# yukw777/EILEV

Hardware: AMD Instinct MI355X
Metric: clips/sec (8-frame, 16 in-context) encode+generate, eilev-blip2-opt-2.7b (higher is better)
Workload: dtype bf16

## Files before the change

eilev_amd/csrc/attention.hip:

```cpp
#include <type_traits>

#include "common.h"
#include <type_traits>
#include <utility>

int g_attn_force_v1 = 0, g_attn_dbg = 0;
#ifdef EILEV_PROBES
extern "C" int eilev_debug_attn_v1(int on) { g_attn_force_v1 = on & 1; g_attn_dbg = on >> 1; return 0; }
#endif

namespace {

template <int DP, bool DROP = false>
__global__ __launch_bounds__(256) void attn_prefill_kernel(const AttnArgs a) {
    constexpr int KD = DP / 32;
    constexpr int DT = DP / 16;
    constexpr int CH = DP / 8;
    constexpr int KSTR = DP * 2 + 16;
    constexpr int VSTR = 64 * 2 + 16;
    __shared__ __attribute__((aligned(16))) char ks_[64 * KSTR];
    __shared__ __attribute__((aligned(16))) char vt_[DP * VSTR];
    __shared__ int msk_[64];

    const int tid = threadIdx.x, lane = tid & 63, wid = tid >> 6;
// ... 157 lines not shown
template <int NWQ, int DB = 3, bool REL = false>
__global__ __launch_bounds__(64 * NWQ) void attn_prefill_v2_kernel(const AttnArgs a) {
    constexpr int KD = 2 * DB;
    constexpr bool SWZ = DB == 2;
    extern __shared__ __attribute__((aligned(16))) char smem[];
    const int RS = DB == 4 ? 272 : a.hd * 2, CH = RS >> 4;
    const int CHS = a.hd >> 3;
    const int T = 64 * RS;
    int *msk = reinterpret_cast<int *>(smem + 4 * T + 256);
    float *rel_lds = reinterpret_cast<float *>(smem + attn_v2_rel_offset(NWQ, a.hd));

    const int tid = threadIdx.x, lane = tid & 63;
    const int wid = __builtin_amdgcn_readfirstlane(tid >> 6);
    const int l31 = lane & 31, hi = lane >> 5;
    const int b = blockIdx.z, h = blockIdx.y;
    const int q0 = (blockIdx.x * NWQ + wid) * 32;
    const int qrow = q0 + l31;
    const int off = a.skv - a.sq;
    const float sl2 = a.scale * 1.44269504088896340736f;

    const bf16 *qp = a.q + (int64_t)b * a.q_bs + (int64_t)h * a.q_hs;
    const bf16 *kp = a.k + (int64_t)b * a.k_bs + (int64_t)h * a.k_hs;
    const bf16 *vp = a.v + (int64_t)b * a.v_bs + (int64_t)h * a.v_hs;

    int kv_end = a.skv;
    if (a.causal) {
        const int last_q = min(a.sq - 1, (int)(blockIdx.x * NWQ + NWQ) * 32 - 1);
        kv_end = min(a.skv, last_q + off + 1);
    }
    const int ntiles = (kv_end + 63) / 64;

    auto stage_in = [&](int buf, int t) {
        const int kv0 = t * 64;
        for (int i = wid; i < 2 * CH; i += NWQ) {
            const bool isv = i >= CH;
            const int pi = isv ? i - CH : i;
            const int pch = pi * 64 + lane, key = pch / CH, cl = pch - key * CH;
            const int c = SWZ ? (cl ^ ((key >> 1) & 7)) : (DB == 4 && cl >= CHS ? CHS - 1 : cl);
            int gk = kv0 + key;
            gk = gk < a.skv ? gk : a.skv - 1;
            const bf16 *src = isv ? vp + (int64_t)gk * a.ldv + c * 8 : kp + (int64_t)gk * a.ldk + c * 8;
            char *dst = smem + buf * 2 * T + (isv ? T : 0) + pi * 1024;
// ... 121 lines not shown
#pragma unroll
                for (int db = 0; db < DB; ++db) {
                    const char *va = vbase + (kb * 32 + 16 * s2) * RS + (SWZ ? 0 : db * 64);
                    const bf16x4 lo = __builtin_amdgcn_ds_read_tr16_b64_v4bf16((lds_bf16x4_t *)(va + (SWZ ? db * 64 : 0)));
                    const bf16x4 hi4 = __builtin_amdgcn_ds_read_tr16_b64_v4bf16((lds_bf16x4_t *)(va + 8 * RS + (SWZ ? (db ^ 1) * 64 : 0)));
                    const bf16x8 vf = {lo[0], lo[1], lo[2], lo[3], hi4[0], hi4[1], hi4[2], hi4[3]};
                    o[db] = __builtin_amdgcn_mfma_f32_32x32x16_bf16(vf, pb, o[db], 0, 0, 0);
                }
            }
        }
    };

    for (int t = 0; t < ntiles; ++t) {
        const int cur = t & 1;
        if (t + 1 < ntiles && !(a.dbg & DBG_ATTN_NO_PREFETCH)) stage_in(cur ^ 1, t + 1);
        if (active && !(a.dbg & DBG_ATTN_NO_COMPUTE)) {
            const int kv0 = t * 64;
            int vis_end = kv_end;
            if (a.causal) vis_end = min(vis_end, min(a.sq - 1, q0 + 31) + off + 1);
            const bool plain = msk[128 + cur] != 0 && (!a.causal || kv0 + 63 <= q0 + off);
            using two = std::integral_constant<int, 2>;
            using one = std::integral_constant<int, 1>;
            if (NWQ > 8 || (DB == 4 && NWQ == 8)) {
                if (kv0 < vis_end) {
                    if (plain) tile_body(one{}, std::false_type{}, cur, kv0);
                    else tile_body(one{}, std::true_type{}, cur, kv0);
                }
                if (kv0 + 32 < vis_end) {
                    if (plain) tile_body(one{}, std::false_type{}, cur, kv0 + 32);
                    else tile_body(one{}, std::true_type{}, cur, kv0 + 32);
// ... 309 lines not shown
}

template <int HD, int NT>
int launch_attn_frame(const AttnArgs &a, hipStream_t s) {
    constexpr int CH = HD / 8;
    constexpr int NPIECE = (NT * 16 * CH + (12 - CH) + 63) / 64;
    constexpr int smem = 3 * NPIECE * 1024;
    const int npairs = a.batch * a.heads;
    const int grid = npairs < eilev_grid_cus() ? npairs : eilev_grid_cus();
    return eilev_launch<attn_frame_kernel<HD, NT>>(dim3(grid), dim3(576), smem, s, a);
}

#include "attn_frame3.h"

template <int NWQ, int DB = 3, bool REL = false>
int launch_attn_v2(const AttnArgs &a, hipStream_t s) {
    size_t smem = attn_v2_rel_offset(NWQ, a.hd) + (REL ? (size_t)(a.rel_n + 2 * ATTN_V2_REL_SLACK) * sizeof(float) : 0);
    const dim3 grid((a.sq + 32 * NWQ - 1) / (32 * NWQ), a.heads, a.batch), block(64 * NWQ);
    return eilev_launch<attn_prefill_v2_kernel<NWQ, DB, REL>>(grid, block, smem, s, a);
}

}

int launch_attention(const AttnArgs &a_in, hipStream_t s) {
    AttnArgs a = a_in;
    a.dbg = g_attn_dbg;
    if (a.batch <= 0 || a.sq <= 0) return EILEV_OK;
    if (!a.q || !a.k || !a.v || !a.o || a.skv <= 0) return EILEV_E_BADARG;
    if ((a.hd & 7) || a.hd > 128 || (a.ldq & 7) || (a.ldk & 7) || (a.ldv & 7) || (a.ldo & 7) || ((uintptr_t)a.o & 15) || (a.q_hs & 7) ||
        (a.k_hs & 7) || (a.v_hs & 7) || (a.o_hs & 7) || (a.q_bs & 7) || (a.k_bs & 7) || (a.v_bs & 7) || (a.o_bs & 7))
        return EILEV_E_UNSUPPORTED;
    if (a.hm) {
        if (a.hd != 88 || a.sq != 257 || a.skv != 257 || a.causal || a.key_mask || a.rel_tab || a.drop_thr || (a.q_hs & 7) || (a.q_bs & 7) ||
// ... 49 lines not shown
```

eilev_amd/csrc/common.h:

```cpp
#pragma once
#include <hip/hip_runtime.h>
#include <stdint.h>

#include <type_traits>

#include "../../include/eilev.h"

typedef __bf16 bf16;
typedef __attribute__((ext_vector_type(8))) __bf16 bf16x8;
typedef __attribute__((ext_vector_type(4))) __bf16 bf16x4;
typedef __attribute__((ext_vector_type(2))) __bf16 bf16x2;
typedef __attribute__((ext_vector_type(4))) float f32x4;
typedef __attribute__((ext_vector_type(16))) float f32x16;

#define EILEV_HIP_CHECK(expr)                          \
    do {                                               \
        hipError_t _e = (expr);                        \
        if (_e != hipSuccess) return (int)_e;          \
    } while (0)

static inline int eilev_num_cu() {
    static int n = 0;
    if (!n) {
        int dev = 0, cu = 0;
// ... 219 lines not shown
    DBG_ATTN_FRAME_STAMPS = 1 << 8,
    DBG_ATTN_FRAME3_STAMPS = 1 << 9,
    DBG_ATTN_HEAD_MAJOR = 1 << 10,
    DBG_ATTN_FRAME3_NO_STORES = 1 << 11,
};
enum GemmForce : int { FORCE_NONE = 0, FORCE_PP4 = 9, FORCE_W6 = 12, FORCE_64x128 = 13, FORCE_128x128 = 14, FORCE_SPLIT_K = 15 };

struct GemmArgs {
    const bf16 *A;
    int64_t lda;
    const bf16 *W;
    int64_t ldw;
    const bf16 *Wp = nullptr;
    int a_frag = 0, c_frag = 0, ln_frag = 0;
    int hm_tok = 0, hm_heads = 0, hm_hd = 0;
    const bf16 *bias;
    const bf16 *resid;
    int64_t ldr;
    void *C;
    int64_t ldc;
    int M, N, K;
    int epi;
    int out_f32;
    float scale;
    int scale_cols;
    int patch_group;
    int dbg;
    float *scratch;
    size_t scratch_bytes;
    const float *wscale = nullptr;
// ... 5 lines not shown
    const float *ln_csum = nullptr;
    float *stat_out = nullptr;
    int64_t stat_ld = 0;
    const bf16 *ln_gamma = nullptr, *ln_beta = nullptr;
    bf16 *ln_out = nullptr;
    float ln_eps = 0.0f;
    int k_slice = 0;
    unsigned long long *trace = nullptr;
    int trace_tiles = 0;
};

__host__ __device__ static inline int64_t frag32_index(int row, int col) { return (int64_t)(col >> 5) * 1024 + row * 32 + (col & 31); }

int launch_gemm(const GemmArgs &g, int prof_kind, hipStream_t s);
bool gemm_rows32_takes(const GemmArgs &g);
int launch_pp4_ext(const GemmArgs &g, int grid, hipStream_t s);
#ifdef EILEV_PROBES
#define EILEV_TRACE_M16 true
#else
#define EILEV_TRACE_M16 false
#endif
static inline bool pp4_all_lean(const GemmArgs &g) {
    const bool scale_ok = g.scale_cols == 0 || (g.scale_cols % 16 == 0 && g.epi == 0 && !g.resid && !g.ln_rows && !g.stat_out);
    return g.N % 128 == 0 && !g.out_f32 && g.patch_group == 0 && scale_ok && !g.wscale && !g.ascale && !g.dbg && (!g.trace || EILEV_TRACE_M16);
}
static inline bool hm_takes(const GemmArgs &g) {
    return g.hm_tok > 0 && g.hm_heads > 0 && g.hm_hd > 64 && g.hm_hd % 8 == 0 && g.N == 3 * g.hm_heads * g.hm_hd && g.ln_rows && g.epi == 0 && !g.resid &&
           !g.stat_out && !g.scale_cols && pp4_all_lean(g) && g.N % 64 == 0 && g.M % g.hm_tok == 0 && (int64_t)g.M * g.N * 2 < 0xfffffff0ll;
}
bool gemv_rows_ok(int M, int N, int K);
int launch_gemv_rows(int pro, const bf16 *x, int64_t ldx, const bf16 *gamma, const bf16 *beta, float eps, const float *part, int heads, int hd,
                     int nsplit, const bf16 *W, const bf16 *bias, const bf16 *resid, int64_t ldr, void *out, int64_t ldo, int out_f32, int M, int N,
                     int K, int epi, float scale, int scale_cols, hipStream_t s);
bool gemv1_ok(int N, int K, int pro);
int launch_gemv1(int pro, const bf16 *x, const bf16 *gamma, const bf16 *beta, float eps, const bf16 *W, const bf16 *bias, const bf16 *resid, void *out,
                 int out_f32, int N, int K, int epi, float scale, int scale_cols, hipStream_t s, const float *part = nullptr, int heads = 0, int hd = 0,
                 int nsplit = 0);
bool gemvm_ok(int M, int N, int K, int pro);
int launch_gemvm(int pro, const bf16 *x, int64_t ldx, const bf16 *gamma, const bf16 *beta, float eps, const bf16 *W, const bf16 *bias, const bf16 *resid,
                 int64_t ldr, void *out, int64_t ldo, int out_f32, int M, int N, int K, int epi, float scale, int scale_cols, hipStream_t s);
int launch_im2col(const void *pix, int dtype, bf16 *out, int64_t rows, int frames, int img, int patch, int kp, hipStream_t s);
int launch_pad_rows(const bf16 *w, bf16 *out, int rows, int k, int kp, hipStream_t s);
int launch_cls_rows(const bf16 *cls, const bf16 *pos, bf16 *x, int64_t frames_total, int tok, int d, hipStream_t s);
int launch_quant_rows_e4m3(const bf16 *x, int64_t ldx, uint8_t *q, float *scale, int64_t rows, int cols, hipStream_t s);
// ... 30 lines not shown
    const bf16 *q, *k, *v;
    bf16 *o;
    int64_t q_bs, k_bs, v_bs, o_bs;
    int64_t q_hs, k_hs, v_hs, o_hs;
    int64_t ldq, ldk, ldv, ldo;
    int batch, heads, sq, skv, hd;
    float scale;
    int causal;
    const int32_t *key_mask;
    int64_t mask_ld;
    int dbg = 0;
    const float *rel_tab = nullptr;
    int64_t rel_hs = 0;
    int rel_off = 0, rel_n = 0;
    int hm = 0;
    uint32_t drop_thr = 0, drop_seed = 0;
    float drop_scale = 1.0f;
};
static inline AttnArgs attn_rows(const bf16 *q, int64_t ldq, const bf16 *k, int64_t ldk, const bf16 *v, int64_t ldv, bf16 *o, int64_t batch,
                                 int64_t heads, int64_t sq, int64_t skv, int64_t hd, float scale) {
    AttnArgs a;
    a.q = q; a.k = k; a.v = v; a.o = o;
    a.q_bs = sq * ldq; a.k_bs = skv * ldk; a.v_bs = skv * ldv; a.o_bs = sq * heads * hd;
    a.q_hs = a.k_hs = a.v_hs = a.o_hs = hd;
    a.ldq = ldq; a.ldk = ldk; a.ldv = ldv; a.ldo = heads * hd;
    a.batch = (int)batch; a.heads = (int)heads; a.sq = (int)sq; a.skv = (int)skv; a.hd = (int)hd; a.scale = scale; a.causal = 0;
    a.key_mask = nullptr; a.mask_ld = 0;
    return a;
}
static inline AttnArgs attn_cache(const bf16 *q, int64_t ldq, const bf16 *kplane, const bf16 *vplane, int64_t cap, bf16 *o, int64_t batch,
// ... 38 lines not shown
```

eilev_amd/csrc/gemm.hip:

```cpp
#include "gemm_common.h"
#include "gemm_tiled.h"
#include "gemm_pp4.h"
#include "gemm_w6.h"
#include "gemm_skinny.h"

int g_eilev_grid_cus = 0;
#ifdef EILEV_PROBES
int g_gemm_debug = 0;
extern "C" int eilev_debug_gemm_flags(int f) { g_gemm_debug = f; return 0; }
extern "C" int eilev_debug_grid_cus(int n) { g_eilev_grid_cus = n; return 0; }
#endif
#ifdef EILEV_PROBES
unsigned long long *g_gemm_trace = nullptr;
int g_gemm_trace_tiles = 0;
extern "C" int eilev_debug_gemm_trace(void *buf, int tiles) { g_gemm_trace = (unsigned long long *)buf; g_gemm_trace_tiles = tiles; return 0; }
#endif

namespace {

#ifndef EILEV_A3_MIN_K
#define EILEV_A3_MIN_K 5120
#endif
bool a3_takes(const GemmArgs &g) { return g.epi == 0 && g.K >= EILEV_A3_MIN_K; }

int launch_pp4(const GemmArgs &g, hipStream_t s) {
    constexpr int smem = PP4_SMEM;
    const int tiles = ((g.M + 255) / 256) * ((g.N + 255) / 256);
    const int ncu = eilev_grid_cus();
    const int grid = tiles < ncu ? tiles : ncu / 8 * 8;
    if (g.A8 || g.ln_rows || g.stat_out) return launch_pp4_ext(g, grid, s);
    if (pp4_all_lean(g) && g.epi != 1) {
        if (a3_takes(g)) return eilev_launch<gemm_pp4_kernel<0, false, 0, 2, true>>(dim3(grid), dim3(512), smem, s, g);
        return eilev_with_epi<0, 2>(g.epi, [&](auto e) { return eilev_launch<gemm_pp4_kernel<decltype(e)::value, false, 0, 2>>(dim3(grid), dim3(512), smem, s, g); });
    }
    return eilev_with_epi<0, 1, 2>(g.epi, [&](auto e) { return eilev_launch<gemm_pp4_kernel<decltype(e)::value>>(dim3(grid), dim3(512), smem, s, g); });
}

constexpr int64_t kOffsetLimit = 0x7fff0000ll;
bool fits_offset(int64_t rows, int64_t ld) { return rows * ld * 2 < kOffsetLimit; }

GemmArgs with_probes(const GemmArgs &g_in) {
    GemmArgs g = g_in;
#ifdef EILEV_PROBES
    g.dbg = g_gemm_debug;
    g.trace = g_gemm_trace;
    g.trace_tiles = g_gemm_trace_tiles;
// ... 27 lines not shown
bool w8_streams(const GemmArgs &g) { return g.M <= 32 && g.K % 256 == 0 && g.patch_group == 0; }
int w8_check(const GemmArgs &g) {
    if (!g.A || !g.C || !g.wscale || g.N <= 0 || g.K <= 0 || g.ldw != g.K || ((uintptr_t)g.W8 & 15) || (g.K & 15)) return EILEV_E_BADARG;
    if (!w8_streams(g) && !g.w8_scratch) return EILEV_E_WORKSPACE;
    return EILEV_OK;
}
int w8_expand(const GemmArgs &g, hipStream_t s) {
    const int64_t n16 = (int64_t)g.N * g.K / 16;
    hipLaunchKernelGGL(w8_expand_kernel, dim3((unsigned)ceil_div64(n16, 256)), dim3(256), 0, s, g.W8, g.w8_scratch, n16);
    EILEV_LAUNCH_CHECK();
    return EILEV_OK;
}

bool ln_fold(const GemmArgs &g) { return g.ln_rows != nullptr || g.stat_out != nullptr; }
bool skinny_dma_ok(const GemmArgs &g) { return g.K % 256 == 0 && (!(g.dbg & DBG_GEMM_SKINNY_NO_DMA) || g.W8); }
bool skinny_takes(const GemmArgs &g) { return (g.M <= 16 || (g.M <= 32 && skinny_dma_ok(g))) && g.patch_group == 0 && !ln_fold(g); }

int check_args(const GemmArgs &g) {
    if (!g.A || !g.W || !g.C || g.N <= 0 || g.K <= 0) return EILEV_E_BADARG;
    if ((g.K & 7) || (g.lda & 7) || (g.ldw & 7) || ((uintptr_t)g.A & 15) || ((uintptr_t)g.W & 15)) return EILEV_E_UNSUPPORTED;
    if (g.hm_tok && (!hm_takes(g) || !fits_offset(g.M, g.lda))) return EILEV_E_UNSUPPORTED;
    if (ln_fold(g) && (g.W8 || g.wscale || g.out_f32 || g.patch_group || g.scale_cols || g.K % BK || !fits_offset(g.N, g.ldw))) return EILEV_E_UNSUPPORTED;
    const bool skinny = skinny_takes(g);
    if ((g.a_frag || g.c_frag || g.ln_frag) && !skinny) return EILEV_E_UNSUPPORTED;
    if (!skinny && !g.out_f32 && ((g.ldc & 7) || (g.N & 3) || ((uintptr_t)g.C & 15) || (g.resid && ((g.ldr & 7) || ((uintptr_t)g.resid & 15))) ||
                                   (g.bias && ((uintptr_t)g.bias & 7))))
        return EILEV_E_UNSUPPORTED;
    return EILEV_OK;
}


// ... 125 lines not shown
}
int launch_split_k(const GemmArgs &g, hipStream_t s) {
    const int tiles = (int)(ceil_div64(g.M, 128) * ceil_div64(g.N, 128)), nk = g.K / BK;
    int slices = 512 / tiles;
    slices = slices < 2 ? 2 : (slices > 16 ? 16 : slices);
    if (slices > nk / 8) slices = nk / 8 > 1 ? nk / 8 : 1;
    GemmArgs gs = g;
    gs.k_slice = (nk + slices - 1) / slices;
    slices = (nk + gs.k_slice - 1) / gs.k_slice;
    EILEV_HIP_CHECK(hipMemsetAsync(g.C, 0, (size_t)g.M * g.ldc * sizeof(float), s));
    return eilev_launch<gemm_glds_kernel<128, 128, 2, 2, 0, 2, 2, 0>>(dim3(tiles, slices), dim3(256), 2 * (128 + 128) * 128, s, gs);
}

bool t64x128_takes(const GemmArgs &g) { return ceil_div64(g.M, 128) * ceil_div64(g.N, 128) < 96 && g.M > 64; }

int launch_wide(const GemmArgs &g, hipStream_t s) {
    const int force = (g.dbg >> DBG_GEMM_FORCE_SHIFT) & 15;
    const bool no_dma = g.dbg & DBG_GEMM_NO_DMA;
    int cfg = tile_cfg(g);
    bool promoted = false;
    if (cfg == CFG_256x128_1S && g.K % BK == 0 && !(g.dbg & DBG_GEMM_NO_WIDE)) cfg = CFG_256x256, promoted = true;
    if (cfg == CFG_256x128 && w6_ok(g) && force == FORCE_NONE && !(g.dbg & (DBG_GEMM_NO_WIDE | DBG_GEMM_NO_W6 | DBG_GEMM_NO_DMA))) cfg = CFG_256x256, promoted = true;
    if (force == FORCE_PP4) cfg = CFG_256x256;
    if (force == FORCE_64x128 || force == FORCE_128x128 || force == FORCE_SPLIT_K) cfg = CFG_128x128;
    else if (force >= CFG_256x256 && force <= CFG_128x128) cfg = force;

    if (w6_ok(g) && (force == FORCE_W6 || (force == FORCE_NONE && cfg == CFG_256x256 && w6_pick(g) && !(g.dbg & (DBG_GEMM_NO_W6 | DBG_GEMM_NO_DMA)))))
        return launch_w6(g, s);
    switch (cfg) {
        case CFG_256x256:
            if (!(promoted && (g.dbg & DBG_GEMM_WIDE_TILED)) && (force == FORCE_NONE || force == FORCE_PP4) && !no_dma && g.K % BK == 0 && fits_offset(g.N, g.ldw))
                return launch_pp4(g, s);
            return launch_tiled<256, 256, 2, 4, 2, 2>(g, s);
        case CFG_256x128_1S: return launch_tiled<256, 128, 4, 2, 1, 4, 1>(g, s);
        case CFG_256x128: return launch_tiled<256, 128, 4, 2, 2, 2>(g, s);
        default:
            if (split_k_takes(g) && (force == FORCE_NONE || force == FORCE_SPLIT_K) && !no_dma) return launch_split_k(g, s);
            if ((force == FORCE_64x128 || (force == FORCE_NONE && t64x128_takes(g))) && g.M > 64 && !no_dma) return launch_tiled<64, 128, 1, 2, 2, 3>(g, s);
            return launch_tiled<128, 128, 2, 2, 2, 2>(g, s);
    }
}

}


static int launch_gemm_core(const GemmArgs &g_in, int prof_kind, hipStream_t s, bool *ln_done);

bool gemm_rows32_takes(const GemmArgs &g) {
    if (!g.A || !g.W || !g.C || g.W8 || g.wscale || g.M <= 16 || g.M > 32 || g.K % 256 || g.patch_group || g.ln_rows || g.stat_out) return false;
    if ((g.lda & 7) || (g.ldw & 7) || ((uintptr_t)g.A & 15) || ((uintptr_t)g.W & 15) || (g.dbg & DBG_GEMM_NO_ROWS32)) return false;
    SkinnyArgs a;
    a.g = g;
    a.mr = 32;
    int ks = 1, ksteps = 0, grid_x = 0;
    return rows32_plan(g, (g.N + 15) / 16, skinny_n_cu(), a, ks, ksteps, grid_x);
}

extern "C" int eilev_stream_layout_pack(const void *w, int64_t n, int64_t k, void *out, void *stream) {
    if (!w || !out || w == out || n < 1 || k < 1) return EILEV_E_BADARG;
    if (n > 0x7fffffff || k > 0x7fffffff || n * k > 0x7fffffff0ll) return EILEV_E_UNSUPPORTED;
    int ks = 0, ksteps = 0, grid_x = 0;
    if (!rows32_shape((int)n, (int)k, skinny_n_cu(), ks, ksteps, grid_x)) return EILEV_E_UNSUPPORTED;
    const int64_t chunks = n * (k >> 3);
    hipLaunchKernelGGL(stream_pack_kernel, dim3((unsigned)((chunks + 255) / 256)), dim3(256), 0, (hipStream_t)stream, (const bf16 *)w, (bf16 *)out, (int)n, (int)k, grid_x);
    EILEV_LAUNCH_CHECK();
    return EILEV_OK;
}

int launch_gemm(const GemmArgs &g, int prof_kind, hipStream_t s) {
    bool ln_done = false;
    const int rc = launch_gemm_core(g, prof_kind, s, &ln_done);
// ... 10 lines not shown
    if (g.W8) {
        const int rc = w8_check(g);
        if (rc != EILEV_OK) return rc;
        if (!w8_streams(g)) {
            const int rc_x = w8_expand(g, s);
            if (rc_x != EILEV_OK) return rc_x;
            GemmArgs e = g_in;
            e.W = g.w8_scratch;
            e.W8 = nullptr;
            return launch_gemm_core(e, prof_kind, s, ln_done);
        }
        g.W = reinterpret_cast<const bf16 *>(g.W8);
    }
    const int rc = check_args(g);
    if (rc != EILEV_OK) return rc;
    if (skinny_takes(g)) return launch_skinny(g, s, ln_done);
    if (const int64_t rows = chunk_rows(g)) return launch_row_chunks(g_in, rows, prof_kind, s);
    return profiled(ln_fold(g) ? launch_pp4 : launch_wide, g, prof_kind, s);
}
```

eilev_amd/csrc/gemm_pp4.h:

```cpp
#pragma once
#include "gemm_common.h"

namespace {

#ifndef EILEV_PP4_DEEP
#define EILEV_PP4_DEEP 1
#endif
template <int EPI, bool F8 = false, int LN = 0, int M16K = 0, bool A3 = false>
__global__ __launch_bounds__(512, 2) void gemm_pp4_kernel(const GemmArgs g) {
    constexpr bool M16 = M16K != 0, HT16 = M16K == 2;
    static_assert(!M16 || !F8, "16 x 16 form: bf16 instances");
    constexpr int BM = 256, BN = 256, NWM = 2, NWN = 4, NW = 8;
    constexpr int WM = BM / NWM, WN = BN / NWN, TM = WM / 32, TN = WN / 32;
    constexpr int STEP = (BM + BN) * 128;
    constexpr int PC = 8;
    static_assert(!A3 || M16, "A3: lean epilogues only");
    constexpr int STG0 = A3 ? 2 * BM * 128 : 2 * STEP;

    extern __shared__ __attribute__((aligned(16))) char smem[];
    auto a_slot = [&](int st) { return smem + (A3 ? (st % 3) * (BM * 128) : (st & 1) * STEP); };
    auto w_slot = [&](int st) { return smem + (A3 ? 3 * (BM * 128) + (st & 1) * (BN * 128) : (st & 1) * STEP + BM * 128); };
    const int tiles_m = (g.M + BM - 1) / BM, tiles_n = (g.N + BN - 1) / BN, ntiles = tiles_m * tiles_n;
    const int tid = threadIdx.x, lane = tid & 63;
    const int wid = __builtin_amdgcn_readfirstlane(tid >> 6);
    const int wm = wid / NWN, wn = wid % NWN;
    const int l31 = lane & 31, hi = lane >> 5;
// ... 229 lines not shown
                } else {
                    const int cph = (HD - 64) >> 3, jb = ((rr - NH * 64) >> 3) + schunk, hh = jb / cph;
                    ent.x = (plane * NH + hh) * TOK * HD + TOK * 64 + (jb - hh * cph) * 8;
                    ent.y = HD - 64;
                }
                const int fw = __builtin_amdgcn_readfirstlane(r0 / TOK);
                const int m0 = r0 + srow, f0 = m0 / TOK;
                hm_t = m0 - f0 * TOK;
                hm_str2 = __builtin_amdgcn_readfirstlane(ent.y * 2);
                hm_off = (unsigned)(((f0 - fw) * TOK * g.N + ent.x + hm_t * ent.y) * 2);
                hm_off_w = hm_off + (unsigned)(TOK * g.N * 2) - (unsigned)(TOK * hm_str2);
                const int64_t left = ((int64_t)g.M / TOK - fw) * TOK * g.N * 2;
                rch = uniform_rsrc(reinterpret_cast<bf16 *>(g.C) + (int64_t)fw * TOK * g.N, (int)(unsigned)(left < 0xfffffff0ll ? left : 0xfffffff0ll));
            }
        }
        u32x4_t rv[4];
        auto res_load = [&](int u) {
#pragma unroll
            for (int it = 0; it < 4; ++it) rv[it] = __builtin_amdgcn_raw_buffer_load_b128(rr, rs_voff, (u * 32 + it * 8) * (int)(g.ldr * 2), 0);
        };
        if constexpr (RES) res_load(0);
        bf16x4 biasr[M16 ? 1 : TN][4];
        bf16x4 biasr16[M16 ? TN16 : 1];
        if constexpr (M16) {
#pragma unroll
            for (int j = 0; j < TN16; ++j) {
                if (g.bias) biasr16[j] = *reinterpret_cast<const bf16x4 *>(g.bias + cn0 + coff + j * 16 + g4 * 4);
                else biasr16[j] = (bf16x4){(bf16)0.f, (bf16)0.f, (bf16)0.f, (bf16)0.f};
            }
        } else {
// ... 125 lines not shown
                }
            } else if constexpr (LNP) {
                typedef __attribute__((ext_vector_type(2))) unsigned u32x2_t;
                const f32x2_t t = (f32x2_t){st1 + __shfl_xor(st1, 32), st2 + __shfl_xor(st2, 32)};
                if (hi == 0) __builtin_amdgcn_raw_buffer_store_b64(__builtin_bit_cast(u32x2_t, t), rst, (U * 32 + l31) * 8, 0, 0);
            }
            __builtin_amdgcn_sched_barrier(0);
            bf16x8 erb[2];
#pragma unroll
            for (int h2 = 0; h2 < 2; ++h2) {
#pragma unroll
                for (int b = 0; b < 2; ++b) {
                    const int row = (h2 * 2 + b) * 8 + srow;
                    erb[b] = *reinterpret_cast<const bf16x8 *>(stg + row * 128 + ((schunk ^ (row & 7)) << 4));
                }
                if (hm) {
                    if constexpr (HMI) {
#pragma unroll
                        for (int b = 0; b < 2; ++b) {
                            const int RO = U * 32 + (h2 * 2 + b) * 8;
                            const unsigned vo = hm_t + RO >= g.hm_tok ? hm_off_w : hm_off;
                            __builtin_amdgcn_raw_buffer_store_b128(__builtin_bit_cast(u32x4_t, erb[b]), rch, vo, RO * hm_str2, EILEV_HM_AUX);
                        }
                    }
                } else {
#pragma unroll
                for (int b = 0; b < 2; ++b)
                    __builtin_amdgcn_raw_buffer_store_b128(__builtin_bit_cast(u32x4_t, erb[b]), rc, st_voff, (U * 32 + (h2 * 2 + b) * 8) * (int)(g.ldc * 2), EILEV_ST_AUX);
                }
            }
            asm volatile("s_nop 1" ::: "memory");
            __builtin_amdgcn_sched_barrier(0);
        });
    };
#define PP_WAIT_LGKM0() __builtin_amdgcn_s_waitcnt(0xC07F)
#define PP_WAIT_LGKM0_VM0() __builtin_amdgcn_s_waitcnt(0x0070)
// ... 265 lines not shown
```

eilev_amd/csrc/misc.hip:

```cpp
#include "common.h"

namespace {

template <typename T>
__global__ void im2col_kernel(const T *__restrict__ pix, bf16 *__restrict__ out, int64_t rows, int frames, int img,
                              int patch, int kp) {
    const int64_t idx = (int64_t)blockIdx.x * blockDim.x + threadIdx.x;
    const int chunks = kp >> 3;
    if (idx >= rows * chunks) return;
    const int64_t row = idx / chunks;
    const int c = (int)(idx - row * chunks);
    const int g = img / patch, gg = g * g, pp = patch * patch;
    const int64_t f = row / gg;
    const int p = (int)(row - f * gg), py = p / g, px = p - py * g;
    const int64_t n = f / frames;
    const int t = (int)(f - n * frames);
    float v[8];
#pragma unroll
    for (int e = 0; e < 8; ++e) {
        const int k = c * 8 + e;
        float val = 0.0f;
        if (k < 3 * pp) {
            const int ch = k / pp, rem = k - ch * pp, dy = rem / patch, dx = rem - dy * patch;
            val = (float)pix[(((n * 3 + ch) * frames + t) * img + py * patch + dy) * (int64_t)img + px * patch + dx];
// ... 667 lines not shown
                     int past) {
    hipLaunchKernelGGL(pos_ids_kernel, dim3(batch), dim3(1024), 0, s, mask, pid, L);
    EILEV_LAUNCH_CHECK();
    hipLaunchKernelGGL(add_pos_kernel, dim3(batch * (L - past)), dim3(256), 0, s, emb, pos, pid, h, d, L - past, L, past);
    EILEV_LAUNCH_CHECK();
    return EILEV_OK;
}
int launch_decode_embed(const bf16 *embed, const bf16 *pos, const int64_t *tokens, const int32_t *n_valid, const int32_t *state,
                        int vocab, int max_pid, bf16 *h, int batch, int d, hipStream_t s) {
    hipLaunchKernelGGL(decode_embed_kernel, dim3(batch), dim3(256), 0, s, embed, pos, tokens, n_valid, state, vocab, max_pid, h, d);
    EILEV_LAUNCH_CHECK();
    return EILEV_OK;
}
int launch_kv_write(const bf16 *qkv, bf16 *kc, bf16 *vc, int batch, int rows_per_b, int heads, int hd, int cap, int seq_len,
                    const int32_t *state, hipStream_t s, int slot0) {
    hipLaunchKernelGGL(kv_write_kernel, dim3(batch * rows_per_b), dim3(256), 0, s, qkv, kc, vc, rows_per_b, heads, hd, cap, seq_len, state, slot0);
    EILEV_LAUNCH_CHECK();
    return EILEV_OK;
}
int launch_topk_logprob(const float *logits, const float *row_score, int rows, int vocab, int keep, float *out_val, int32_t *out_idx, hipStream_t s) {
    if (vocab > 65536 || (vocab & 3) || keep < 1 || keep > 64 || (((uintptr_t)logits) & 15)) return EILEV_E_UNSUPPORTED;
    hipLaunchKernelGGL(topk_logprob_kernel, dim3(rows), dim3(1024), 0, s, logits, row_score, vocab, keep, out_val, out_idx);
    EILEV_LAUNCH_CHECK();
    return EILEV_OK;
}
int launch_beam_advance(const float *row_lp, const int32_t *row_tok, int batch, int beams, int keep, int max_new, const int32_t *state,
                        const int64_t *eos_ids, int n_eos, const float *len_pow, int recip, int early, int64_t *run_seq, float *run_score,
                        int64_t *fin_seq, float *fin_score, int64_t *fin_len, uint8_t *finished, uint8_t *can_improve, int64_t *tokens, int32_t *anc,
                        int gen_cap, int64_t *scratch, hipStream_t s) {
    if (beams * keep > 2048 || keep > 64 || beams > 32 || (anc && gen_cap * beams > 32 * 64) || n_eos > 8) return EILEV_E_UNSUPPORTED;
    BeamAdvanceArgs a;
// ... 210 lines not shown
```

eilev_amd/csrc/opt.hip:

```cpp
#include "stages.h"

namespace {
inline int64_t opt_ws_rows(int64_t M) { return (M > 16 && M < 32) ? 32 : M; }

struct OptBufs {
    bf16 *h, *x, *att, *qkv, *ffn;
    int32_t *pid;
    float *scratch;
    uint8_t *a8;
    float *a8_scale;
    size_t used;
};

OptBufs carve_opt(const EilevDims *d, int64_t M, void *ws) {
    Carver cv{(char *)ws};
    OptBufs b;
    M = opt_ws_rows(M);
    b.h = cv.take<bf16>((size_t)M * d->t_hidden);
    b.x = cv.take<bf16>((size_t)M * d->t_hidden);
    b.att = cv.take<bf16>((size_t)M * d->t_hidden);
    b.qkv = cv.take<bf16>((size_t)M * 3 * d->t_hidden);
    b.ffn = cv.take<bf16>((size_t)M * d->t_ffn);
    b.pid = cv.take<int32_t>((size_t)M);
    b.scratch = cv.take<float>(kSkinnyScratch / sizeof(float));
// ... 23 lines not shown
        g.W8 = w8;
        g.wscale = sc;
        g.ldw = g.K;
        return EILEV_OK;
    }
    if (g.M > 32 || g.K % 256 != 0) {
        if (!w->w8_expand || w->w8_expand_bytes < (size_t)g.N * g.K * sizeof(bf16)) return EILEV_E_WORKSPACE;
        g.w8_scratch = (bf16 *)w->w8_expand;
    }
    g.W8 = w8;
    g.wscale = sc;
    g.ldw = g.K;
    return EILEV_OK;
}

int opt_qkv(const EilevDims *d, const EilevOptWeights *w, int l, const OptBufs &b, int64_t M, hipStream_t s, int a_frag = 0) {
    const EilevOptLayer *L = &w->layers[l];
    const int D = d->t_hidden;
    const float scaling = 1.0f / sqrtf((float)(D / d->t_heads));
    const void *ws[3] = {L->q_w, L->k_w, L->v_w}, *bs[3] = {L->q_b, L->k_b, L->v_b};
    const bool bias_fused = packed(bs, 3, D);
    if (w->layers_w8) {
        if (!bias_fused && (L->q_b || L->k_b || L->v_b)) return EILEV_E_UNSUPPORTED;
        GemmArgs g = sk_gemm(b.scratch, b.x, D, nullptr, D, L->q_b, nullptr, 0, b.qkv, 3 * D, M, 3 * D, D, 0);
        g.scale = scaling; g.scale_cols = D;
        RC(use_w8(g, w, w->layers_w8[l].qkv_w8, w->layers_w8[l].qkv_scale, b, s));
        return launch_gemm(g, 5, s);
    }
    const bool fused = packed(ws, 3, (size_t)D * D) && bias_fused;
    for (int i = 0; i < (fused ? 1 : 3); ++i) {
        GemmArgs g = sk_gemm(b.scratch, b.x, D, ws[i], D, bs[i], nullptr, 0, b.qkv + i * D, 3 * D, M, fused ? 3 * D : D, D, 0);
        if (i == 0) { g.scale = scaling; g.scale_cols = D; }
        if (fused && w->layers_stream && M > 16 && M <= 32) g.Wp = (const bf16 *)w->layers_stream[l].qkv_s;
        g.a_frag = a_frag;
        RC(launch_gemm(g, 5, s));
    }
    return EILEV_OK;
}

int opt_tail(const EilevDims *d, const EilevOptWeights *w, int l, const OptBufs &b, int64_t M, hipStream_t s, const void *next_ln_w = nullptr,
             const void *next_ln_b = nullptr, int frag = 0, bool dry = false) {
    const EilevOptLayer *L = &w->layers[l];
    const EilevOptLayerW8 *Q = w->layers_w8 ? &w->layers_w8[l] : nullptr;
    const int D = d->t_hidden, Ft = d->t_ffn;
    const EilevOptLayerStream *S = (w->layers_stream && !Q && M > 16 && M <= 32) ? &w->layers_stream[l] : nullptr;
    GemmArgs g = sk_gemm(b.scratch, b.att, D, L->o_w, D, L->o_b, b.h, D, b.h, D, M, D, D, 0);
    g.ln_gamma = (const bf16 *)L->ln2_w; g.ln_beta = (const bf16 *)L->ln2_b; g.ln_out = b.x; g.ln_eps = d->t_eps;
    if (S) g.Wp = (const bf16 *)S->o_s;
    g.a_frag = g.ln_frag = frag;
// ... 6 lines not shown
    if (dry && !gemm_rows32_takes(g)) return EILEV_E_UNSUPPORTED;
    if (Q) RC(use_w8(g, w, Q->fc1_w8, Q->fc1_scale, b, s));
    if (!dry) RC(launch_gemm(g, 5, s));
    g = sk_gemm(b.scratch, b.ffn, Ft, L->fc2_w, Ft, L->fc2_b, b.h, D, b.h, D, M, D, Ft, 0);
    if (S) g.Wp = (const bf16 *)S->fc2_s;
    if (next_ln_w) {
        g.ln_gamma = (const bf16 *)next_ln_w; g.ln_beta = (const bf16 *)next_ln_b; g.ln_out = b.x; g.ln_eps = d->t_eps;
    }
    g.a_frag = frag;
    g.ln_frag = next_ln_w ? frag : 0;
    if (dry) return gemm_rows32_takes(g) ? EILEV_OK : EILEV_E_UNSUPPORTED;
    if (Q) RC(use_w8(g, w, Q->fc2_w8, Q->fc2_scale, b, s));
    return launch_gemm(g, 5, s);
}

int g_decode_frag = 1;
}
int g_decode_rows = 1;
#ifdef EILEV_PROBES
extern "C" int eilev_debug_decode_rows(int on) { g_decode_rows = on; return 0; }
extern "C" int eilev_debug_decode_frag(int on) { g_decode_frag = on; return 0; }
#endif
namespace {

bool opt_qkv_packed(const EilevDims *d, const EilevOptWeights *w) {
    const int D = d->t_hidden;
    for (int l = 0; l < d->t_layers; ++l) {
        const EilevOptLayer *L = &w->layers[l];
        const void *ws[3] = {L->q_w, L->k_w, L->v_w}, *bs[3] = {L->q_b, L->k_b, L->v_b};
        if (!packed(ws, 3, (size_t)D * D) || !L->q_b || !packed(bs, 3, D)) return false;
// ... 98 lines not shown
        const EilevOptLayer *L = &w->layers[l];
        DecodeAttnArgs al = at_block(a, l, kv_layer, gen_layer);
        al.out_frag = frag;
        if (l == 0) RC(launch_layernorm(b.h, D, (const bf16 *)L->ln1_w, (const bf16 *)L->ln1_b, b.x, D, M, D, d->t_eps, s));
        RC(opt_qkv(d, w, l, b, M, s, l > 0 ? frag : 0));
        RC(launch_attn_decode(al, s));
        const bool last = l + 1 == d->t_layers;
        RC(opt_tail(d, w, l, b, M, s, last ? w->final_ln_w : w->layers[l + 1].ln1_w, last ? w->final_ln_b : w->layers[l + 1].ln1_b, frag));
    }
    GemmArgs g = opt_lm_head(d, w, b, M, logits);
    g.a_frag = frag;
    return launch_gemm(g, 5, s);
}

int opt_blocks(const EilevDims *d, const EilevOptWeights *w, const OptBufs &b, const void *inputs_embeds, const int32_t *attn_mask, int64_t batch,
               int64_t rows, int64_t past_len, bool from_cache, void *kv_cache, int64_t kv_capacity, void *hidden, hipStream_t s) {
    const int D = d->t_hidden, H = d->t_heads, hd = D / H;
    const int64_t M = batch * rows, total = past_len + rows;
    RC(launch_pos_embed((const bf16 *)inputs_embeds, (const bf16 *)w->embed_positions, attn_mask, b.pid, b.h, (int)batch, (int)total, D,
                        s, (int)past_len));
    const KvCache kv(batch, D, kv_capacity);
    const size_t hs_bytes = (size_t)M * D * sizeof(bf16);
    for (int l = 0; l < d->t_layers; ++l) {
        const EilevOptLayer *L = &w->layers[l];
        bf16 *kc = kv.k((bf16 *)kv_cache, l), *vc = kv.v((bf16 *)kv_cache, l);
        if (hidden) RC(copy_hidden(hidden, l, b.h, hs_bytes, s));
        RC(launch_layernorm(b.h, D, (const bf16 *)L->ln1_w, (const bf16 *)L->ln1_b, b.x, D, M, D, d->t_eps, s));
        RC(opt_qkv(d, w, l, b, M, s));
        RC(launch_kv_write(b.qkv, kc, vc, (int)batch, (int)rows, H, hd, (int)kv_capacity, (int)total, nullptr, s, (int)past_len));
        AttnArgs a = from_cache ? attn_cache(b.qkv, 3 * D, kc, vc, kv_capacity, b.att, batch, H, rows, total, hd, 1.0f)
                                : attn_rows(b.qkv, 3 * D, b.qkv + D, 3 * D, b.qkv + 2 * D, 3 * D, b.att, batch, H, rows, total, hd, 1.0f);
        a.causal = 1; a.key_mask = attn_mask; a.mask_ld = total;
        RC(launch_attention(a, s));
        RC(opt_tail(d, w, l, b, M, s));
    }
    RC(launch_layernorm(b.h, D, (const bf16 *)w->final_ln_w, (const bf16 *)w->final_ln_b, b.x, D, M, D, d->t_eps, s));
    if (hidden) RC(copy_hidden(hidden, d->t_layers, b.x, hs_bytes, s));
    return EILEV_OK;
}

int opt_prefill_impl(const EilevDims *d, const EilevOptWeights *w, const void *inputs_embeds, const int32_t *attn_mask, int64_t batch,
                     int64_t seq_len, void *kv_cache, int64_t kv_capacity, float *logits_last, float *logits_all, void *hidden,
                     void *workspace, size_t workspace_bytes, void *stream) {
    if (!d || !w || !inputs_embeds || !attn_mask || !kv_cache || !workspace || batch <= 0 || seq_len <= 0) return EILEV_E_BADARG;
    if (seq_len > kv_capacity || seq_len > d->max_pos) return EILEV_E_BADARG;
    if (!dims_ok_opt(d)) return EILEV_E_UNSUPPORTED;
    if (workspace_bytes < eilev_opt_workspace_bytes(d, batch, seq_len)) return EILEV_E_WORKSPACE;
    hipStream_t s = (hipStream_t)stream;
    const int D = d->t_hidden;
    const int64_t M = batch * seq_len;
    const OptBufs b = carve_opt(d, M, workspace);
    RC(opt_blocks(d, w, b, inputs_embeds, attn_mask, batch, seq_len, 0, false, kv_cache, kv_capacity, hidden, s));
    if (logits_all) {
        GemmArgs g = mk_gemm(b.x, D, w->embed_tokens, D, nullptr, nullptr, 0, logits_all, d->vocab, M, d->vocab, D, 0);
        g.out_f32 = 1;
        RC(launch_gemm(g, 5, s));
    }
    if (logits_last) {
        GemmArgs g = sk_gemm(b.scratch, b.x + (seq_len - 1) * (int64_t)D, seq_len * (int64_t)D, w->embed_tokens, D, nullptr, nullptr, 0,
                             logits_last, d->vocab, batch, d->vocab, D, 0);
        g.out_f32 = 1;
        RC(launch_gemm(g, 5, s));
    }
    return EILEV_OK;
}
}

// ... 155 lines not shown
```

Before: 231.7.

## Fuse KV-cache write into QKV GEMM and compute last layer only for final row

Adds a KVC epilogue to the pp4 QKV GEMM that writes the K and V planes straight into the KV cache, so prefill no longer needs the separate kv_write kernel. In the last OPT layer it runs attention only for the final query block and does out-proj, LN2 and the FFN only on each sample's last row, since only last-row logits are needed. The attention kernel also zeroes masked K/V rows in LDS, because values now come from the cache, and it gains a query-block offset. In exchange it adds complex eligibility checks and a new GEMM instance, and it risks correctness because cache rows are read directly.

Result: no change. 232.4 (median of 6 runs) (+0.3%).

```diff
diff --git a/eilev_amd/csrc/attention.hip b/eilev_amd/csrc/attention.hip
--- a/eilev_amd/csrc/attention.hip
+++ b/eilev_amd/csrc/attention.hip
@@ -195,7 +195,8 @@
     const int wid = __builtin_amdgcn_readfirstlane(tid >> 6);
     const int l31 = lane & 31, hi = lane >> 5;
     const int b = blockIdx.z, h = blockIdx.y;
-    const int q0 = (blockIdx.x * NWQ + wid) * 32;
+    const int qblk = blockIdx.x + a.qb0;
+    const int q0 = (qblk * NWQ + wid) * 32;
     const int qrow = q0 + l31;
     const int off = a.skv - a.sq;
     const float sl2 = a.scale * 1.44269504088896340736f;
@@ -206,7 +207,7 @@
 
     int kv_end = a.skv;
     if (a.causal) {
-        const int last_q = min(a.sq - 1, (int)(blockIdx.x * NWQ + NWQ) * 32 - 1);
+        const int last_q = min(a.sq - 1, (qblk * NWQ + NWQ) * 32 - 1);
         kv_end = min(a.skv, last_q + off + 1);
     }
     const int ntiles = (kv_end + 63) / 64;
@@ -358,6 +359,17 @@
     for (int t = 0; t < ntiles; ++t) {
         const int cur = t & 1;
         if (t + 1 < ntiles && !(a.dbg & DBG_ATTN_NO_PREFETCH)) stage_in(cur ^ 1, t + 1);
+        if (msk[128 + cur] == 0) {
+            char *kt = smem + cur * 2 * T;
+            for (int i = tid; i < 64 * CH; i += 64 * NWQ) {
+                const int key = i / CH, c16 = (i - key * CH) * 16;
+                if (!msk[cur * 64 + key]) {
+                    *reinterpret_cast<uint4 *>(kt + key * RS + c16) = make_uint4(0, 0, 0, 0);
+                    *reinterpret_cast<uint4 *>(kt + T + key * RS + c16) = make_uint4(0, 0, 0, 0);
+                }
+            }
+            __syncthreads();
+        }
         if (active && !(a.dbg & DBG_ATTN_NO_COMPUTE)) {
             const int kv0 = t * 64;
             int vis_end = kv_end;
@@ -697,9 +709,12 @@
 #include "attn_frame3.h"
 
 template <int NWQ, int DB = 3, bool REL = false>
-int launch_attn_v2(const AttnArgs &a, hipStream_t s) {
+int launch_attn_v2(const AttnArgs &a_in, hipStream_t s) {
+    AttnArgs a = a_in;
+    const int qblocks = (a.sq + 32 * NWQ - 1) / (32 * NWQ);
+    a.qb0 = a.last_q_only ? qblocks - 1 : 0;
     size_t smem = attn_v2_rel_offset(NWQ, a.hd) + (REL ? (size_t)(a.rel_n + 2 * ATTN_V2_REL_SLACK) * sizeof(float) : 0);
-    const dim3 grid((a.sq + 32 * NWQ - 1) / (32 * NWQ), a.heads, a.batch), block(64 * NWQ);
+    const dim3 grid(qblocks - a.qb0, a.heads, a.batch), block(64 * NWQ);
     return eilev_launch<attn_prefill_v2_kernel<NWQ, DB, REL>>(grid, block, smem, s, a);
 }
 
diff --git a/eilev_amd/csrc/common.h b/eilev_amd/csrc/common.h
--- a/eilev_amd/csrc/common.h
+++ b/eilev_amd/csrc/common.h
@@ -257,6 +257,9 @@
     const bf16 *Wp = nullptr;
     int a_frag = 0, c_frag = 0, ln_frag = 0;
     int hm_tok = 0, hm_heads = 0, hm_hd = 0;
+    bf16 *kvc_k = nullptr, *kvc_v = nullptr;
+    int kvc_rows = 0, kvc_cap = 0, kvc_heads = 0, kvc_hd = 0;
+    int family_pp4 = 0;
     const bf16 *bias;
     const bf16 *resid;
     int64_t ldr;
@@ -292,6 +295,7 @@
 
 int launch_gemm(const GemmArgs &g, int prof_kind, hipStream_t s);
 bool gemm_rows32_takes(const GemmArgs &g);
+bool gemm_wide_on_pp4(const GemmArgs &g);
 int launch_pp4_ext(const GemmArgs &g, int grid, hipStream_t s);
 #ifdef EILEV_PROBES
 #define EILEV_TRACE_M16 true
@@ -306,6 +310,13 @@
     return g.hm_tok > 0 && g.hm_heads > 0 && g.hm_hd > 64 && g.hm_hd % 8 == 0 && g.N == 3 * g.hm_heads * g.hm_hd && g.ln_rows && g.epi == 0 && !g.resid &&
            !g.stat_out && !g.scale_cols && pp4_all_lean(g) && g.N % 64 == 0 && g.M % g.hm_tok == 0 && (int64_t)g.M * g.N * 2 < 0xfffffff0ll;
 }
+static inline bool kvc_takes(const GemmArgs &g) {
+    const int64_t w = (int64_t)g.kvc_heads * g.kvc_hd;
+    return g.kvc_k && g.kvc_v && g.kvc_heads > 0 && g.kvc_hd > 0 && g.kvc_hd % 8 == 0 && w % 64 == 0 && g.N == 3 * w && g.kvc_rows >= 128 &&
+           g.kvc_rows <= g.kvc_cap && g.M % g.kvc_rows == 0 && g.epi == 0 && !g.resid && !g.ln_rows && !g.stat_out && !g.ln_out && !g.hm_tok &&
+           pp4_all_lean(g) && 2 * w * g.kvc_cap * 2 < 0xfffffff0ll;
+}
+bool gemm_kvc_takes(const GemmArgs &g);
 bool gemv_rows_ok(int M, int N, int K);
 int launch_gemv_rows(int pro, const bf16 *x, int64_t ldx, const bf16 *gamma, const bf16 *beta, float eps, const float *part, int heads, int hd,
                      int nsplit, const bf16 *W, const bf16 *bias, const bf16 *resid, int64_t ldr, void *out, int64_t ldo, int out_f32, int M, int N,
@@ -366,6 +377,7 @@
     int64_t rel_hs = 0;
     int rel_off = 0, rel_n = 0;
     int hm = 0;
+    int last_q_only = 0, qb0 = 0;
     uint32_t drop_thr = 0, drop_seed = 0;
     float drop_scale = 1.0f;
 };
diff --git a/eilev_amd/csrc/gemm.hip b/eilev_amd/csrc/gemm.hip
--- a/eilev_amd/csrc/gemm.hip
+++ b/eilev_amd/csrc/gemm.hip
@@ -30,6 +30,7 @@
     const int grid = tiles < ncu ? tiles : ncu / 8 * 8;
     if (g.A8 || g.ln_rows || g.stat_out) return launch_pp4_ext(g, grid, s);
     if (pp4_all_lean(g) && g.epi != 1) {
+        if (g.kvc_k) return eilev_launch<gemm_pp4_kernel<0, false, 0, 2, false, true>>(dim3(grid), dim3(512), smem, s, g);
         if (a3_takes(g)) return eilev_launch<gemm_pp4_kernel<0, false, 0, 2, true>>(dim3(grid), dim3(512), smem, s, g);
         return eilev_with_epi<0, 2>(g.epi, [&](auto e) { return eilev_launch<gemm_pp4_kernel<decltype(e)::value, false, 0, 2>>(dim3(grid), dim3(512), smem, s, g); });
     }
@@ -87,7 +88,7 @@
 
 bool ln_fold(const GemmArgs &g) { return g.ln_rows != nullptr || g.stat_out != nullptr; }
 bool skinny_dma_ok(const GemmArgs &g) { return g.K % 256 == 0 && (!(g.dbg & DBG_GEMM_SKINNY_NO_DMA) || g.W8); }
-bool skinny_takes(const GemmArgs &g) { return (g.M <= 16 || (g.M <= 32 && skinny_dma_ok(g))) && g.patch_group == 0 && !ln_fold(g); }
+bool skinny_takes(const GemmArgs &g) { return !g.family_pp4 && (g.M <= 16 || (g.M <= 32 && skinny_dma_ok(g))) && g.patch_group == 0 && !ln_fold(g); }
 
 int check_args(const GemmArgs &g) {
     if (!g.A || !g.W || !g.C || g.N <= 0 || g.K <= 0) return EILEV_E_BADARG;
@@ -243,7 +244,8 @@
 
 bool t64x128_takes(const GemmArgs &g) { return ceil_div64(g.M, 128) * ceil_div64(g.N, 128) < 96 && g.M > 64; }
 
-int launch_wide(const GemmArgs &g, hipStream_t s) {
+enum WideKernel : int { WK_W6, WK_PP4, WK_256x256, WK_256x128_1S, WK_256x128, WK_SPLIT_K, WK_64x128, WK_128x128 };
+WideKernel wide_kernel(const GemmArgs &g) {
     const int force = (g.dbg >> DBG_GEMM_FORCE_SHIFT) & 15;
     const bool no_dma = g.dbg & DBG_GEMM_NO_DMA;
     int cfg = tile_cfg(g);
@@ -255,19 +257,41 @@
     else if (force >= CFG_256x256 && force <= CFG_128x128) cfg = force;
 
     if (w6_ok(g) && (force == FORCE_W6 || (force == FORCE_NONE && cfg == CFG_256x256 && w6_pick(g) && !(g.dbg & (DBG_GEMM_NO_W6 | DBG_GEMM_NO_DMA)))))
-        return launch_w6(g, s);
+        return WK_W6;
     switch (cfg) {
         case CFG_256x256:
             if (!(promoted && (g.dbg & DBG_GEMM_WIDE_TILED)) && (force == FORCE_NONE || force == FORCE_PP4) && !no_dma && g.K % BK == 0 && fits_offset(g.N, g.ldw))
-                return launch_pp4(g, s);
-            return launch_tiled<256, 256, 2, 4, 2, 2>(g, s);
-        case CFG_256x128_1S: return launch_tiled<256, 128, 4, 2, 1, 4, 1>(g, s);
-        case CFG_256x128: return launch_tiled<256, 128, 4, 2, 2, 2>(g, s);
+                return WK_PP4;
+            return WK_256x256;
+        case CFG_256x128_1S: return WK_256x128_1S;
+        case CFG_256x128: return WK_256x128;
         default:
-            if (split_k_takes(g) && (force == FORCE_NONE || force == FORCE_SPLIT_K) && !no_dma) return launch_split_k(g, s);
-            if ((force == FORCE_64x128 || (force == FORCE_NONE && t64x128_takes(g))) && g.M > 64 && !no_dma) return launch_tiled<64, 128, 1, 2, 2, 3>(g, s);
-            return launch_tiled<128, 128, 2, 2, 2, 2>(g, s);
-    }
+            if (split_k_takes(g) && (force == FORCE_NONE || force == FORCE_SPLIT_K) && !no_dma) return WK_SPLIT_K;
+            if ((force == FORCE_64x128 || (force == FORCE_NONE && t64x128_takes(g))) && g.M > 64 && !no_dma) return WK_64x128;
+            return WK_128x128;
+    }
+}
+int launch_wide(const GemmArgs &g, hipStream_t s) {
+    switch (wide_kernel(g)) {
+        case WK_W6: return launch_w6(g, s);
+        case WK_PP4: return launch_pp4(g, s);
+        case WK_256x256: return launch_tiled<256, 256, 2, 4, 2, 2>(g, s);
+        case WK_256x128_1S: return launch_tiled<256, 128, 4, 2, 1, 4, 1>(g, s);
+        case WK_256x128: return launch_tiled<256, 128, 4, 2, 2, 2>(g, s);
+        case WK_SPLIT_K: return launch_split_k(g, s);
+        case WK_64x128: return launch_tiled<64, 128, 1, 2, 2, 3>(g, s);
+        default: return launch_tiled<128, 128, 2, 2, 2, 2>(g, s);
+    }
+}
+
+bool pp4_family_ok(const GemmArgs &g) {
+    return !g.A8 && !g.W8 && !ln_fold(g) && g.patch_group == 0 && g.K % BK == 0 && fits_offset(g.N, g.ldw) && !g.a_frag && !g.c_frag && !g.ln_frag &&
+           !g.out_f32;
+}
+
+bool kvc_launch_ok(const GemmArgs &g) {
+    return kvc_takes(g) && !a3_takes(g) && !g.family_pp4 && pp4_family_ok(g) && check_args(g) == EILEV_OK && !skinny_takes(g) && !chunk_rows(g) &&
+           wide_kernel(g) == WK_PP4;
 }
 
 }
@@ -284,6 +308,14 @@
     int ks = 1, ksteps = 0, grid_x = 0;
     return rows32_plan(g, (g.N + 15) / 16, skinny_n_cu(), a, ks, ksteps, grid_x);
 }
+
+bool gemm_wide_on_pp4(const GemmArgs &g_in) {
+    const GemmArgs g = with_probes(g_in);
+    if (g.M <= 0 || g.family_pp4 || !pp4_family_ok(g) || check_args(g) != EILEV_OK || skinny_takes(g) || chunk_rows(g)) return false;
+    return wide_kernel(g) == WK_PP4;
+}
+
+bool gemm_kvc_takes(const GemmArgs &g) { return kvc_launch_ok(with_probes(g)); }
 
 extern "C" int eilev_stream_layout_pack(const void *w, int64_t n, int64_t k, void *out, void *stream) {
     if (!w || !out || w == out || n < 1 || k < 1) return EILEV_E_BADARG;
@@ -324,6 +356,8 @@
     }
     const int rc = check_args(g);
     if (rc != EILEV_OK) return rc;
+    if (g.kvc_k && !kvc_launch_ok(g)) return EILEV_E_UNSUPPORTED;
+    if (g.family_pp4) return pp4_family_ok(g) ? profiled(launch_pp4, g, prof_kind, s) : EILEV_E_UNSUPPORTED;
     if (skinny_takes(g)) return launch_skinny(g, s, ln_done);
     if (const int64_t rows = chunk_rows(g)) return launch_row_chunks(g_in, rows, prof_kind, s);
     return profiled(ln_fold(g) ? launch_pp4 : launch_wide, g, prof_kind, s);
diff --git a/eilev_amd/csrc/gemm_pp4.h b/eilev_amd/csrc/gemm_pp4.h
--- a/eilev_amd/csrc/gemm_pp4.h
+++ b/eilev_amd/csrc/gemm_pp4.h
@@ -6,10 +6,11 @@
 #ifndef EILEV_PP4_DEEP
 #define EILEV_PP4_DEEP 1
 #endif
-template <int EPI, bool F8 = false, int LN = 0, int M16K = 0, bool A3 = false>
+template <int EPI, bool F8 = false, int LN = 0, int M16K = 0, bool A3 = false, bool KVC = false>
 __global__ __launch_bounds__(512, 2) void gemm_pp4_kernel(const GemmArgs g) {
     constexpr bool M16 = M16K != 0, HT16 = M16K == 2;
     static_assert(!M16 || !F8, "16 x 16 form: bf16 instances");
+    static_assert(!KVC || (M16 && LN == 0 && EPI == 0 && !A3), "KVC: the plain 16 x 16 bias-only instance");
     constexpr int BM = 256, BN = 256, NWM = 2, NWN = 4, NW = 8;
     constexpr int WM = BM / NWM, WN = BN / NWN, TM = WM / 32, TN = WN / 32;
     constexpr int STEP = (BM + BN) * 128;
@@ -269,6 +270,27 @@
                 rch = uniform_rsrc(reinterpret_cast<bf16 *>(g.C) + (int64_t)fw * TOK * g.N, (int)(unsigned)(left < 0xfffffff0ll ? left : 0xfffffff0ll));
             }
         }
+        constexpr bool KVI = KVC && !RES;
+        bool kvc = false;
+        if constexpr (KVI) {
+            const int D1 = g.N / 3, n0 = cn0 + coff;
+            const int plane = __builtin_amdgcn_readfirstlane(n0 / D1);
+            kvc = plane > 0;
+            if (kvc) {
+                const int TOK = g.kvc_rows, HD = g.kvc_hd;
+                const int col = n0 - plane * D1 + schunk * 8, hh = col / HD;
+                const int64_t sample = (int64_t)g.kvc_heads * g.kvc_cap * HD;
+                const int fw = __builtin_amdgcn_readfirstlane(r0 / TOK);
+                const int m0 = r0 + srow, f0 = m0 / TOK;
+                hm_t = m0 - f0 * TOK;
+                hm_str2 = __builtin_amdgcn_readfirstlane(HD * 2);
+                hm_off = (unsigned)(f0 - fw) * (unsigned)(sample * 2) + (unsigned)(((hh * g.kvc_cap + hm_t) * HD + (col - hh * HD)) * 2);
+                hm_off_w = hm_off + (unsigned)(sample * 2) - (unsigned)(TOK * hm_str2);
+                int64_t left = ((int64_t)g.M / TOK - fw) * sample * 2;
+                left = left < 0 ? 0 : (left < 0xfffffff0ll ? left : 0xfffffff0ll);
+                rch = uniform_rsrc((plane == 1 ? g.kvc_k : g.kvc_v) + (int64_t)fw * sample, (int)(unsigned)left);
+            }
+        }
         u32x4_t rv[4];
         auto res_load = [&](int u) {
 #pragma unroll
@@ -424,12 +446,12 @@
                     const int row = (h2 * 2 + b) * 8 + srow;
                     erb[b] = *reinterpret_cast<const bf16x8 *>(stg + row * 128 + ((schunk ^ (row & 7)) << 4));
                 }
-                if (hm) {
-                    if constexpr (HMI) {
+                if (hm || kvc) {
+                    if constexpr (HMI || KVI) {
 #pragma unroll
                         for (int b = 0; b < 2; ++b) {
                             const int RO = U * 32 + (h2 * 2 + b) * 8;
-                            const unsigned vo = hm_t + RO >= g.hm_tok ? hm_off_w : hm_off;
+                            const unsigned vo = hm_t + RO >= (KVI ? g.kvc_rows : g.hm_tok) ? hm_off_w : hm_off;
                             __builtin_amdgcn_raw_buffer_store_b128(__builtin_bit_cast(u32x4_t, erb[b]), rch, vo, RO * hm_str2, EILEV_HM_AUX);
                         }
                     }
diff --git a/eilev_amd/csrc/misc.hip b/eilev_amd/csrc/misc.hip
--- a/eilev_amd/csrc/misc.hip
+++ b/eilev_amd/csrc/misc.hip
@@ -705,7 +705,9 @@
 }
 int launch_kv_write(const bf16 *qkv, bf16 *kc, bf16 *vc, int batch, int rows_per_b, int heads, int hd, int cap, int seq_len,
                     const int32_t *state, hipStream_t s, int slot0) {
+    prof_begin(7, 4.0 * batch * (double)rows_per_b * heads * hd * sizeof(bf16), s);
     hipLaunchKernelGGL(kv_write_kernel, dim3(batch * rows_per_b), dim3(256), 0, s, qkv, kc, vc, rows_per_b, heads, hd, cap, seq_len, state, slot0);
+    prof_end(s);
     EILEV_LAUNCH_CHECK();
     return EILEV_OK;
 }
diff --git a/eilev_amd/csrc/opt.hip b/eilev_amd/csrc/opt.hip
--- a/eilev_amd/csrc/opt.hip
+++ b/eilev_amd/csrc/opt.hip
@@ -61,7 +61,8 @@
     return EILEV_OK;
 }
 
-int opt_qkv(const EilevDims *d, const EilevOptWeights *w, int l, const OptBufs &b, int64_t M, hipStream_t s, int a_frag = 0) {
+int opt_qkv(const EilevDims *d, const EilevOptWeights *w, int l, const OptBufs &b, int64_t M, hipStream_t s, int a_frag = 0, bf16 *kc = nullptr,
+            bf16 *vc = nullptr, int64_t rows = 0, int64_t cap = 0, bool *kv_done = nullptr) {
     const EilevOptLayer *L = &w->layers[l];
     const int D = d->t_hidden;
     const float scaling = 1.0f / sqrtf((float)(D / d->t_heads));
@@ -80,6 +81,11 @@
         if (i == 0) { g.scale = scaling; g.scale_cols = D; }
         if (fused && w->layers_stream && M > 16 && M <= 32) g.Wp = (const bf16 *)w->layers_stream[l].qkv_s;
         g.a_frag = a_frag;
+        if (fused && kc && vc && kv_done && rows <= 0x7fffffff && cap <= 0x7fffffff) {
+            GemmArgs gk = g;
+            gk.kvc_k = kc; gk.kvc_v = vc; gk.kvc_rows = (int)rows; gk.kvc_cap = (int)cap; gk.kvc_heads = d->t_heads; gk.kvc_hd = D / d->t_heads;
+            if (gemm_kvc_takes(gk)) { g = gk; *kv_done = true; }
+        }
         RC(launch_gemm(g, 5, s));
     }
     return EILEV_OK;
@@ -116,6 +122,28 @@
     return launch_gemm(g, 5, s);
 }
 
+int opt_tail_last_rows(const EilevDims *d, const EilevOptWeights *w, int l, const OptBufs &b, int64_t batch, int64_t rows, hipStream_t s, bool dry) {
+    const EilevOptLayer *L = &w->layers[l];
+    const int D = d->t_hidden, Ft = d->t_ffn;
+    const int64_t M = batch * rows, ld = rows * D, last = (rows - 1) * D;
+    GemmArgs out = sk_gemm(b.scratch, b.att, D, L->o_w, D, L->o_b, b.h, D, b.h, D, M, D, D, 0);
+    GemmArgs fc1 = sk_gemm(b.scratch, b.x, D, L->fc1_w, D, L->fc1_b, nullptr, 0, b.ffn, Ft, M, Ft, D, 2);
+    GemmArgs fc2 = sk_gemm(b.scratch, b.ffn, Ft, L->fc2_w, Ft, L->fc2_b, b.h, D, b.h, D, M, D, Ft, 0);
+    if (dry) {
+        if (w->layers_w8 || batch > 0x7fffffff / rows || 256 * ld * 2 >= 0x7fff0000ll) return EILEV_E_UNSUPPORTED;
+        return gemm_wide_on_pp4(out) && gemm_wide_on_pp4(fc1) && gemm_wide_on_pp4(fc2) ? EILEV_OK : EILEV_E_UNSUPPORTED;
+    }
+    out.A = b.att + last; out.lda = ld; out.resid = b.h + last; out.ldr = ld; out.C = b.h + last; out.ldc = ld;
+    fc1.A = b.x + last; fc1.lda = ld;
+    fc2.resid = b.h + last; fc2.ldr = ld; fc2.C = b.h + last; fc2.ldc = ld;
+    out.M = fc1.M = fc2.M = (int)batch;
+    out.family_pp4 = fc1.family_pp4 = fc2.family_pp4 = 1;
+    RC(launch_gemm(out, 5, s));
+    RC(launch_layernorm(b.h + last, ld, (const bf16 *)L->ln2_w, (const bf16 *)L->ln2_b, b.x + last, ld, batch, D, d->t_eps, s));
+    RC(launch_gemm(fc1, 5, s));
+    return launch_gemm(fc2, 5, s);
+}
+
 int g_decode_frag = 1;
 }
 int g_decode_rows = 1;
@@ -244,23 +272,34 @@
 }
 
 int opt_blocks(const EilevDims *d, const EilevOptWeights *w, const OptBufs &b, const void *inputs_embeds, const int32_t *attn_mask, int64_t batch,
-               int64_t rows, int64_t past_len, bool from_cache, void *kv_cache, int64_t kv_capacity, void *hidden, hipStream_t s) {
+               int64_t rows, int64_t past_len, bool from_cache, void *kv_cache, int64_t kv_capacity, void *hidden, hipStream_t s,
+               bool last_only = false) {
     const int D = d->t_hidden, H = d->t_heads, hd = D / H;
     const int64_t M = batch * rows, total = past_len + rows;
     RC(launch_pos_embed((const bf16 *)inputs_embeds, (const bf16 *)w->embed_positions, attn_mask, b.pid, b.h, (int)batch, (int)total, D,
                         s, (int)past_len));
     const KvCache kv(batch, D, kv_capacity);
     const size_t hs_bytes = (size_t)M * D * sizeof(bf16);
+    last_only = last_only && !hidden && !from_cache && opt_tail_last_rows(d, w, d->t_layers - 1, b, batch, rows, s, true) == EILEV_OK;
     for (int l = 0; l < d->t_layers; ++l) {
         const EilevOptLayer *L = &w->layers[l];
         bf16 *kc = kv.k((bf16 *)kv_cache, l), *vc = kv.v((bf16 *)kv_cache, l);
         if (hidden) RC(copy_hidden(hidden, l, b.h, hs_bytes, s));
         RC(launch_layernorm(b.h, D, (const bf16 *)L->ln1_w, (const bf16 *)L->ln1_b, b.x, D, M, D, d->t_eps, s));
-        RC(opt_qkv(d, w, l, b, M, s));
-        RC(launch_kv_write(b.qkv, kc, vc, (int)batch, (int)rows, H, hd, (int)kv_capacity, (int)total, nullptr, s, (int)past_len));
-        AttnArgs a = from_cache ? attn_cache(b.qkv, 3 * D, kc, vc, kv_capacity, b.att, batch, H, rows, total, hd, 1.0f)
+        bool kv_done = false;
+        const bool fuse_kv = !from_cache && !hidden && past_len == 0;
+        RC(opt_qkv(d, w, l, b, M, s, 0, fuse_kv ? kc : nullptr, vc, rows, kv_capacity, &kv_done));
+        if (!kv_done) RC(launch_kv_write(b.qkv, kc, vc, (int)batch, (int)rows, H, hd, (int)kv_capacity, (int)total, nullptr, s, (int)past_len));
+        AttnArgs a = (from_cache || kv_done) ? attn_cache(b.qkv, 3 * D, kc, vc, kv_capacity, b.att, batch, H, rows, total, hd, 1.0f)
                                 : attn_rows(b.qkv, 3 * D, b.qkv + D, 3 * D, b.qkv + 2 * D, 3 * D, b.att, batch, H, rows, total, hd, 1.0f);
         a.causal = 1; a.key_mask = attn_mask; a.mask_ld = total;
+        if (last_only && l + 1 == d->t_layers) {
+            a.last_q_only = 1;
+            RC(launch_attention(a, s));
+            RC(opt_tail_last_rows(d, w, l, b, batch, rows, s, false));
+            const int64_t ld = rows * D, last = (rows - 1) * D;
+            return launch_layernorm(b.h + last, ld, (const bf16 *)w->final_ln_w, (const bf16 *)w->final_ln_b, b.x + last, ld, batch, D, d->t_eps, s);
+        }
         RC(launch_attention(a, s));
         RC(opt_tail(d, w, l, b, M, s));
     }
@@ -280,7 +319,7 @@
     const int D = d->t_hidden;
     const int64_t M = batch * seq_len;
     const OptBufs b = carve_opt(d, M, workspace);
-    RC(opt_blocks(d, w, b, inputs_embeds, attn_mask, batch, seq_len, 0, false, kv_cache, kv_capacity, hidden, s));
+    RC(opt_blocks(d, w, b, inputs_embeds, attn_mask, batch, seq_len, 0, false, kv_cache, kv_capacity, hidden, s, !logits_all && !hidden));
     if (logits_all) {
         GemmArgs g = mk_gemm(b.x, D, w->embed_tokens, D, nullptr, nullptr, 0, logits_all, d->vocab, M, d->vocab, D, 0);
         g.out_f32 = 1;
```
